# sczhou/CodeFormer

Measured on NVIDIA H100. Metric: faces_per_sec_512x512_batch32, higher is better.
Workload: dtype f32 (split-fp16 operands on tensor cores, fp32 accumulate)

## Files before the change

codeformer_b200/_lib.py:

```python
import ctypes
import os
from ctypes import POINTER, Structure, c_char_p, c_double, c_float, c_int, c_int32, c_int64, c_void_p

_HERE = os.path.dirname(os.path.abspath(__file__))
LIB_PATH = os.path.join(_HERE, 'libcfb200.so')


class CfbConfig(Structure):
    _fields_ = [('kind', c_int32), ('img_size', c_int32), ('nf', c_int32), ('n_ch_mult', c_int32),
                ('ch_mult', c_int32 * 8), ('res_blocks', c_int32), ('n_attn_res', c_int32),
                ('attn_res', c_int32 * 4), ('codebook_size', c_int32), ('emb_dim', c_int32), ('beta', c_float),
                ('dim_embd', c_int32), ('n_head', c_int32), ('n_layers', c_int32), ('latent_size', c_int32),
                ('n_connect', c_int32), ('connect', c_int32 * 6)]


_P = c_void_p
SIGNATURES = {
    'cfb_version': (c_int, []),
    'cfb_last_error': (c_char_p, []),
    'cfb_device_info': (c_int, [POINTER(c_int), POINTER(c_int), POINTER(c_int)]),
    'cfb_net_create': (c_void_p, [POINTER(CfbConfig)]),
    'cfb_net_destroy': (None, [_P]),
    'cfb_net_set_param': (c_int, [_P, c_char_p, _P, c_int64]),
    'cfb_net_prepare': (c_int, [_P, _P]),
# ... 54 lines not shown
    'cfb_retinaface_priors': (c_int64, [c_int32, c_int32]),
    'cfb_retinaface_create': (c_void_p, []),
    'cfb_retinaface_destroy': (None, [_P]),
    'cfb_retinaface_set_param': (c_int, [_P, c_char_p, _P, c_int64]),
    'cfb_retinaface_prepare': (c_int, [_P, _P]),
    'cfb_retinaface_workspace_bytes': (c_int64, [_P, c_int32, c_int32, c_int32]),
    'cfb_retinaface_forward': (c_int, [_P, _P, _P, _P, _P, c_int32, c_int32, c_int32, _P, c_int64, _P]),
    'cfb_retinaface_forward_u8': (c_int, [_P, _P, _P, _P, _P, c_int32, c_int32, c_int32, _P, c_int64, _P]),
    'cfb_retinaface_candidates': (c_int, [_P, _P, _P, c_int32, c_int32, c_int32, c_float, _P, _P, _P]),
    'cfb_yolov5face_predictions': (c_int64, [c_int32, c_int32]),
    'cfb_yolov5face_create': (c_void_p, []),
    'cfb_yolov5face_destroy': (None, [_P]),
    'cfb_yolov5face_set_param': (c_int, [_P, c_char_p, _P, c_int64]),
    'cfb_yolov5face_prepare': (c_int, [_P, _P]),
    'cfb_yolov5face_workspace_bytes': (c_int64, [_P, c_int32, c_int32, c_int32]),
    'cfb_yolov5face_forward': (c_int, [_P, _P, _P, _P, _P, _P, c_int32, c_int32, c_int32, _P, c_int64, _P]),
    'cfb_yolov5face_forward_u8': (c_int, [_P, _P, c_int32, c_int32, c_int32, c_int32, _P, _P, _P, _P, c_int32, c_int32, c_int32,
                                          _P, c_int64, _P]),
    'cfb_yolov5face_candidates': (c_int, [_P, c_int32, c_int32, c_int32, c_float, _P, _P, _P]),
    'cfb_check_async_status': (c_int, []),
    'cfb_debug_set_wait_limit': (c_int, [c_int64]),
    'cfb_debug_inject_fault': (c_int, [c_int32]),
    'cfb_debug_set_stamps': (c_int, [_P]),
    'cfb_nchw_to_nhwc': (c_int, [_P, _P, c_int32, c_int32, c_int32, _P]),
    'cfb_nhwc_to_nchw': (c_int, [_P, _P, c_int32, c_int32, c_int32, _P]),
    'cfb_warp_affine_u8': (c_int, [_P, c_int32, c_int32, _P, c_int32, _P, c_int32, c_int32, c_int32, c_int32, c_int32, c_int32, _P]),
    'cfb_resize_linear_u8': (c_int, [_P, c_int32, c_int32, c_int32, _P, c_int32, c_int32, _P]),
    'cfb_paste_faces_workspace_bytes': (c_int64, [c_int32, c_int32, c_int32, c_int32, c_int32, _P]),
    'cfb_paste_faces': (c_int, [_P, c_int32, c_int32, _P, c_int32, c_int32, _P, _P, c_double, _P, _P, _P, c_int64, _P]),
}

_lib = None


def load():
    global _lib
    if _lib is not None:
        return _lib
    if not os.path.exists(LIB_PATH):
        try:
            from . import build as _build
            _build.build(force=False)
        except Exception as e:
            raise RuntimeError(f'{LIB_PATH} is missing and could not be built with nvcc ({e}); there is no CPU or '
                               'PyTorch fallback for this path -- run `python -m codeformer_b200.build`') from e
    override = os.environ.get('CFB_LIB')
# ... 22 lines not shown
```

codeformer_b200/csrc/conv_tc.cu:

```cuda

#include <cuda.h>
#include <cuda_fp16.h>
#include <cuda_runtime.h>
#include <stdint.h>

#include <stdlib.h>

#include <atomic>
#include <mutex>

#include "conv_tc.cuh"

namespace cfb {

__global__ void tc_absmax_kernel(const float* __restrict__ w, int64_t total, unsigned* __restrict__ slot) {
  float m = 0.f;
  for (int64_t i = (int64_t)blockIdx.x * blockDim.x + threadIdx.x; i < total; i += (int64_t)gridDim.x * blockDim.x)
    m = fmaxf(m, fabsf(w[i]));
#pragma unroll
  for (int o = 16; o > 0; o >>= 1) m = fmaxf(m, __shfl_xor_sync(0xffffffffu, m, o));
  if ((threadIdx.x & 31) == 0) atomicMax(slot, __float_as_uint(m));
}

__global__ void tc_split_weights_kernel(const float* __restrict__ w, __half* __restrict__ hi, __half* __restrict__ lo,
// ... 241 lines not shown
  asm volatile(
      "cp.async.bulk.tensor.4d.shared::cluster.global.mbarrier::complete_tx::bytes [%0], [%1, {%3, %4, %5, %6}], [%2];"
      ::"r"(dst), "l"(map), "r"(bar), "r"(c0), "r"(c1), "r"(c2), "r"(c3)
      : "memory");
}
__device__ __forceinline__ void tma_load_3d(uint32_t dst, const CUtensorMap* map, uint32_t bar, int c0, int c1, int c2) {
  asm volatile(
      "cp.async.bulk.tensor.3d.shared::cluster.global.mbarrier::complete_tx::bytes [%0], [%1, {%3, %4, %5}], [%2];"
      ::"r"(dst), "l"(map), "r"(bar), "r"(c0), "r"(c1), "r"(c2)
      : "memory");
}
__device__ __forceinline__ bool elect_one() {
  uint32_t pred;
  asm volatile(
      "{\n\t.reg .b32 rx;\n\t.reg .pred px;\n\t"
      "elect.sync rx|px, 0xffffffff;\n\t"
      "selp.b32 %0, 1, 0, px;\n\t}"
      : "=r"(pred));
  return pred != 0;
}

__device__ __forceinline__ uint64_t wg_desc(uint32_t saddr, uint32_t sbo) {
  return (uint64_t)((saddr >> 4) & 0x3FFFu) | ((uint64_t)1 << 16) | ((uint64_t)((sbo >> 4) & 0x3FFFu) << 32) | ((uint64_t)1 << 62);
}
__device__ __forceinline__ void wg_fence() { asm volatile("wgmma.fence.sync.aligned;" ::: "memory"); }
__device__ __forceinline__ void wg_commit() { asm volatile("wgmma.commit_group.sync.aligned;" ::: "memory"); }
__device__ __forceinline__ void wg_wait_all() { asm volatile("wgmma.wait_group.sync.aligned 0;" ::: "memory"); }
__device__ __forceinline__ void wg_mma_64x64(float (&d)[32], uint64_t da, uint64_t db, uint32_t accum) {
  asm volatile(
      "{\n\t.reg .pred p;\n\t"
      "setp.ne.b32 p, %34, 0;\n\t"
      "wgmma.mma_async.sync.aligned.m64n64k16.f32.f16.f16 "
      "{%0, %1, %2, %3, %4, %5, %6, %7, %8, %9, %10, %11, %12, %13, %14, %15, "
      "%16, %17, %18, %19, %20, %21, %22, %23, %24, %25, %26, %27, %28, %29, %30, %31}, %32, %33, p, 1, 1, 0, 0;\n\t}"
      : "+f"(d[0]), "+f"(d[1]), "+f"(d[2]), "+f"(d[3]), "+f"(d[4]), "+f"(d[5]), "+f"(d[6]), "+f"(d[7]), "+f"(d[8]),
        "+f"(d[9]), "+f"(d[10]), "+f"(d[11]), "+f"(d[12]), "+f"(d[13]), "+f"(d[14]), "+f"(d[15]), "+f"(d[16]),
        "+f"(d[17]), "+f"(d[18]), "+f"(d[19]), "+f"(d[20]), "+f"(d[21]), "+f"(d[22]), "+f"(d[23]), "+f"(d[24]),
        "+f"(d[25]), "+f"(d[26]), "+f"(d[27]), "+f"(d[28]), "+f"(d[29]), "+f"(d[30]), "+f"(d[31])
      : "l"(da), "l"(db), "r"(accum)
      : "memory");
}

__device__ __forceinline__ void wg_mma_64x128(float (&d)[64], uint64_t da, uint64_t db, uint32_t accum) {
  asm volatile(
      "{\n\t.reg .pred p;\n\t"
      "setp.ne.b32 p, %66, 0;\n\t"
// ... 158 lines not shown
  int in_act;
  const float* bias;
  const float* residual;
  int out_act;
  const float* sft_dec;
  const float* sft_scale;
  float sft_w;
  const float* wscale_inv;
  float* out;
  __half* pl_hi;
  __half* pl_lo;
  float* gn_part;
  int gn_cpg;
#if CFB_TC_STAMPS
  long long* dbg;
#endif
};
#if CFB_TC_STAMPS
#define TC_STAMP(i) do { if (p.dbg != nullptr && blockIdx.x == 0) p.dbg[i] = clock64(); } while (0)
#else
#define TC_STAMP(i) do { } while (0)
#endif

constexpr int XF_SKEW = 128;
constexpr int TC_A_BYTES = 128 * 128;

template <int BN>
struct TcCfg {
  static_assert(BN == 64 || BN == 128, "the wgmma engine runs 64- or 128-wide n-tiles");
  static constexpr bool WIDE = BN == 128;
  static constexpr int MMA_WARPS = WIDE ? 8 : 4;
  static constexpr int EPI_WARPS = WIDE ? 4 : 8;
  static constexpr int THREADS = 32 * (MMA_WARPS + 1 + EPI_WARPS);
  static constexpr int B_BYTES = BN * 128;
  static constexpr int STAGE_BYTES = 2 * TC_A_BYTES + 2 * B_BYTES;
  static constexpr int STAGES = 3;
  static constexpr int SLOT_PITCH = BN + 4;
  static constexpr int SLOT_BYTES = 128 * SLOT_PITCH * 4;
  static constexpr int SLOTS = 1;
  static constexpr int STG_BYTES = WIDE ? 0 : 8 * 4096;
  static constexpr int TAIL_BYTES = SLOT_BYTES + 1024  + 512  + STG_BYTES;
  static constexpr int SMEM_BYTES = STAGES * STAGE_BYTES + TAIL_BYTES;
  static constexpr int H_A_PLANE = 23 * 1024;
  static constexpr int H_A_SLOT = 2 * H_A_PLANE;
  static constexpr int H_A_SLOTS = 2;
  static constexpr int H_B_SLOT = 2 * B_BYTES;
  static constexpr int H_B_SLOTS = WIDE ? 2 : 4;
  static constexpr int H_SMEM_BYTES = H_A_SLOTS * H_A_SLOT + H_B_SLOTS * H_B_SLOT + TAIL_BYTES;
  static constexpr int XF_WARPS = WIDE ? 2 : 4;
  static constexpr int XF_THREADS = THREADS + 32 * XF_WARPS + 32;
  static constexpr int X_A_SLOTS = 2;
  static constexpr int X_A_PLANE2 = H_A_PLANE + XF_SKEW;
  static constexpr int X_B_SLOTS = H_B_SLOTS;
  static constexpr int X_SMEM_BYTES = X_A_SLOTS * H_A_SLOT + X_B_SLOTS * H_B_SLOT + TAIL_BYTES;
};

template <int BN, int CPG, bool HALO, bool XF, bool GEN = false, bool K1 = false, bool CM = false, bool SILU = false>
__global__ void __launch_bounds__(XF ? TcCfg<BN>::XF_THREADS : TcCfg<BN>::THREADS, 1)
conv_tc_kernel(const __grid_constant__ CUtensorMap tmA_hi, const __grid_constant__ CUtensorMap tmA_lo,
               const __grid_constant__ CUtensorMap tmB_hi, const __grid_constant__ CUtensorMap tmB_lo, const TcParams p) {
  static_assert(!XF || HALO, "the fused operand transform exists for the halo engine only");
  static_assert(!GEN || (XF && CPG == 0), "the generalised addressing exists for the fused-transform engine only");
  static_assert(!K1 || (XF && !GEN && CPG == 0), "K1 = fused transform of a 1x1 conv (patch = tile): its own instantiation");
  using Cfg = TcCfg<BN>;
  constexpr bool WIDE = Cfg::WIDE;
  static_assert(!WIDE || (HALO && !GEN && !K1 && CPG != 2), "128-wide tiles exist for the 3x3 / Upsample halo engine");
  static_assert(!CM || (BN == 64 && HALO && !GEN && !K1), "channel-major tiles exist for the 64-channel 3x3 / Upsample halo convs");
  constexpr int MMA_WARPS = Cfg::MMA_WARPS, EPI_WARPS = Cfg::EPI_WARPS;
  constexpr int A_SLOTS = XF ? Cfg::X_A_SLOTS : Cfg::H_A_SLOTS;
  constexpr int STAGES = Cfg::STAGES;
// ... 2 lines not shown
  const int tile_step = (int)gridDim.x;
  extern __shared__ uint8_t smem_raw[];
  uint8_t* smem = reinterpret_cast<uint8_t*>((reinterpret_cast<uintptr_t>(smem_raw) + 1023) & ~(uintptr_t)1023);
  constexpr int NRING = HALO ? (XF ? Cfg::X_B_SLOTS : Cfg::H_B_SLOTS) : STAGES;
  constexpr int RING_BYTES = HALO ? Cfg::H_B_SLOT : STAGE_BYTES;
  uint8_t* ring_base = HALO ? smem + A_SLOTS * Cfg::H_A_SLOT : smem;
  float* acc_slot = reinterpret_cast<float*>(ring_base + NRING * RING_BYTES);
  uint64_t* bars = reinterpret_cast<uint64_t*>(ring_base + NRING * RING_BYTES + Cfg::SLOT_BYTES);
  uint64_t* full = bars;
  uint64_t* empty = bars + NRING;
  uint64_t* cfull = bars + 2 * NRING;
  uint64_t* cempty = bars + 2 * NRING + Cfg::SLOTS;
  uint64_t* afull = bars + 2 * NRING + 2 * Cfg::SLOTS;
  uint64_t* aempty = afull + 3;
  uint64_t* araw = aempty + 3;
  uint8_t* stage_buf = reinterpret_cast<uint8_t*>(bars) + 512;

  constexpr int NWARPS = (XF ? Cfg::XF_THREADS : Cfg::THREADS) / 32;
  const int pwarp = __shfl_sync(0xffffffffu, (int)(threadIdx.x >> 5), 0);
  const int ridx = NWARPS - 1 - pwarp;
  const int warp = pwarp < MMA_WARPS ? 1 : (ridx == 0 ? 0 : ridx + 1);
  const int lane = threadIdx.x & 31;
  bool aborted = false;
  if (threadIdx.x == 0) TC_STAMP(0);

  if (warp == 0 && lane == 0) {
    for (int a = 0; a < 3; ++a) {
      mbar_init(smem_u32(afull + a), XF ? Cfg::XF_WARPS : 1);
      mbar_init(smem_u32(aempty + a), MMA_WARPS);
      mbar_init(smem_u32(araw + a), 1);
    }
    asm volatile("prefetch.tensormap [%0];" ::"l"(&tmA_hi) : "memory");
    asm volatile("prefetch.tensormap [%0];" ::"l"(&tmA_lo) : "memory");
    asm volatile("prefetch.tensormap [%0];" ::"l"(&tmB_hi) : "memory");
    asm volatile("prefetch.tensormap [%0];" ::"l"(&tmB_lo) : "memory");
    for (int s = 0; s < NRING; ++s) { mbar_init(smem_u32(full + s), 1); mbar_init(smem_u32(empty + s), MMA_WARPS); }
    for (int a = 0; a < Cfg::SLOTS; ++a) {
      mbar_init(smem_u32(cfull + a), MMA_WARPS);
      mbar_init(smem_u32(cempty + a), EPI_WARPS);
    }
    asm volatile("fence.mbarrier_init.release.cluster;" ::: "memory");
  }
  __syncthreads();
  pdl_launch_dependents();
  pdl_wait();
  if (threadIdx.x == 0) TC_STAMP(1);

  const int total_tiles = p.m_tiles * p.n_tiles;
  const int nk = p.taps * p.kblocks;

  if (warp == 0) {
    {
      int stage = 0;
      uint32_t phase = 0;
      int aslot = 0;
      uint32_t aphase = 0;
      for (int tile = first_tile; tile < total_tiles; tile += tile_step) {
        const int mt = tile / p.n_tiles, nt = tile - mt * p.n_tiles;
        const int mtl = p.up4 ? (mt >> 2) : mt;
        const int par_y = p.up4 ? ((mt & 3) >> 1) : 0, par_x = p.up4 ? (mt & 1) : 0;
        const int per_img = p.tiles_x * p.tiles_y;
        const int n = mtl / per_img;
        const int rem = mtl - n * per_img;
        const int ty = rem / p.tiles_x, tx = rem - ty * p.tiles_x;
        const int y0 = ty * p.BH * p.stride, x0 = tx * p.BW * p.stride;
        if constexpr (HALO) {
          for (int kb = 0; kb < p.kblocks; ++kb) {
            if constexpr (!XF) {
              mbar_wait<500>(smem_u32(aempty + aslot), aphase ^ 1, aborted); if (aborted) goto teardown;
              if (elect_one()) {
                const uint32_t sa = smem_u32(smem + aslot * Cfg::H_A_SLOT);
                const uint32_t ab = smem_u32(afull + aslot);
                mbar_expect_tx(ab, (uint32_t)(2 * p.PW * p.PH * 128));
                tma_load_4d(sa, &tmA_hi, ab, kb * 64, x0 - p.pad, y0 - p.pad, n);
                tma_load_4d(sa + Cfg::H_A_PLANE, &tmA_lo, ab, kb * 64, x0 - p.pad, y0 - p.pad, n);
              }
              __syncwarp();
              if (++aslot == A_SLOTS) { aslot = 0; aphase ^= 1; }
            }
            for (int tap = 0; tap < p.taps; ++tap) {
              const int btap = p.up4 ? (mt & 3) * 4 + tap : tap;
              mbar_wait<500>(smem_u32(empty + stage), phase ^ 1, aborted); if (aborted) goto teardown;
              if (elect_one()) {
                if (tile == first_tile && tap == 0 && kb == 0) TC_STAMP(2);
                const uint32_t sb = smem_u32(ring_base + stage * RING_BYTES);
                const uint32_t fb = smem_u32(full + stage);
                const bool drop = p.fault && blockIdx.x == 0 && tile == first_tile && kb == 0 && tap == 0;
                mbar_expect_tx(fb, (uint32_t)Cfg::H_B_SLOT);
                if (!drop) tma_load_3d(sb, &tmB_hi, fb, kb * 64, nt * BN, btap);
                tma_load_3d(sb + Cfg::B_BYTES, &tmB_lo, fb, kb * 64, nt * BN, btap);
              }
              __syncwarp();
              if (++stage == NRING) { stage = 0; phase ^= 1; }
            }
          }
        } else {
          for (int tap = 0; tap < p.taps; ++tap) {
            int r, s, btap = tap;
            if (p.up4) { r = (tap >> 1) + par_y; s = (tap & 1) + par_x; btap = (mt & 3) * 4 + tap; }
            else { r = (p.taps == 9) ? tap / 3 : 0; s = (p.taps == 9) ? tap - r * 3 : 0; }
            for (int kb = 0; kb < p.kblocks; ++kb) {
              mbar_wait<500>(smem_u32(empty + stage), phase ^ 1, aborted); if (aborted) goto teardown;
              if (elect_one()) {
                if (tile == first_tile && tap == 0 && kb == 0) TC_STAMP(2);
                const uint32_t sa = smem_u32(smem + stage * STAGE_BYTES);
                const int hh = p.heads > 1 ? n % p.heads : 0, nimg = p.heads > 1 ? n / p.heads : n;
                const int a_img = p.a_img_per_head ? n : nimg;
                const int ac = p.a_c0 + hh * p.a_c_head + kb * 64, bc = p.b_c0 + hh * p.b_c_head + kb * 64;
                const int brow = nt * BN + hh * p.b_r_head;
                const int b3 = p.b_batched ? nimg : btap;
                const uint32_t fb = smem_u32(full + stage);
                const bool drop = p.fault && blockIdx.x == 0 && tile == first_tile && kb == 0 && tap == 0;
                mbar_expect_tx(fb, (uint32_t)Cfg::STAGE_BYTES);
                tma_load_4d(sa, &tmA_hi, fb, ac, x0 + s - p.pad, y0 + r - p.pad, a_img);
                tma_load_4d(sa + TC_A_BYTES, &tmA_lo, fb, ac, x0 + s - p.pad, y0 + r - p.pad, a_img);
                if (!drop) tma_load_3d(sa + 2 * TC_A_BYTES, &tmB_hi, fb, bc, brow, b3);
                tma_load_3d(sa + 2 * TC_A_BYTES + Cfg::B_BYTES, &tmB_lo, fb, bc, brow, b3);
              }
              __syncwarp();
              if (++stage == STAGES) { stage = 0; phase ^= 1; }
            }
          }
        }
      }
    }
  } else if (warp == 1) {
    {
      constexpr bool N128 = WIDE || CM;
      constexpr int MH = N128 ? 1 : 2;
      const uint32_t a_sbo = HALO ? (uint32_t)(p.PW * 128) : 1024u;
      const uint32_t a_half = HALO ? (uint32_t)(8 * p.PW * 128) : 8192u;
      const int wq = (int)(threadIdx.x >> 5) & 3;
      const int wg = (int)(threadIdx.x >> 7);
      const uint32_t bar_id = 2u + (uint32_t)wg;
      const uint32_t slot_base = smem_u32(acc_slot);
      int stage = 0;
      uint32_t phase = 0;
      int slot = 0;
      uint32_t slot_phase = 0;
      int aslot = 0;
      uint32_t aphase = 0;
      float acc[MH][N128 ? 64 : 32];
      if constexpr (N128) {
        for (int tile = first_tile; tile < total_tiles; tile += tile_step) {
          const int par = p.up4 ? ((tile / p.n_tiles) & 3) : 0;
          const int par_y = par >> 1, par_x = par & 1;
          for (int c0 = 0; c0 < nk; c0 += p.chunk) {
            const int c1 = min(c0 + p.chunk, nk);
            uint32_t prev_empty = 0, prev_aempty = 0;
            for (int it = c0; it < c1; ++it) {
              const int kb = it / p.taps;
              const int tap = it - kb * p.taps;
              if (tap == 0) {
                mbar_wait(smem_u32(afull + aslot), aphase, aborted);
                if (wg_any(aborted, bar_id)) { wg_wait_all(); aborted = true; goto teardown; }
              }
              int r = (p.taps == 9) ? tap / 3 : 0;
              int sft = (p.taps == 9) ? tap - r * 3 : 0;
              if (p.up4) { r = (tap >> 1) + par_y; sft = (tap & 1) + par_x; }
              const uint32_t a_hi0 = smem_u32(smem + aslot * Cfg::H_A_SLOT) + (uint32_t)((r * p.PW + sft) * 128) +
                                     (uint32_t)wg * a_half;
              const uint32_t a_lo0 = a_hi0 + (uint32_t)(XF ? Cfg::X_A_PLANE2 : Cfg::H_A_PLANE);
              const uint32_t bsm = smem_u32(ring_base + stage * RING_BYTES);
              mbar_wait(smem_u32(full + stage), phase, aborted);
              if (wg_any(aborted, bar_id)) { wg_wait_all(); aborted = true; goto teardown; }
              wg_fence();
#pragma unroll
              for (int k = 0; k < 4; ++k) {
                const uint64_t db_hi = wg_desc(bsm + 32 * k, 1024u), db_lo = wg_desc(bsm + Cfg::B_BYTES + 32 * k, 1024u);
                const uint64_t da_hi = wg_desc(a_hi0 + 32 * k, a_sbo), da_lo = wg_desc(a_lo0 + 32 * k, a_sbo);
                if constexpr (CM) {
                  wg_mma_64x128(acc[0], db_hi, da_lo, (it == c0 && k == 0) ? 0u : 1u);
                  wg_mma_64x128(acc[0], db_lo, da_hi, 1u);
                  wg_mma_64x128(acc[0], db_hi, da_hi, 1u);
                } else {
                  wg_mma_64x128(acc[0], da_lo, db_hi, (it == c0 && k == 0) ? 0u : 1u);
                  wg_mma_64x128(acc[0], da_hi, db_lo, 1u);
                  wg_mma_64x128(acc[0], da_hi, db_hi, 1u);
                }
              }
              wg_commit();
              wg_wait_1();
              __syncwarp();
              mbar_arrive_if(prev_empty, lane == 0 && prev_empty != 0);
              mbar_arrive_if(prev_aempty, lane == 0 && prev_aempty != 0);
              prev_empty = smem_u32(empty + stage);
              prev_aempty = tap == p.taps - 1 ? smem_u32(aempty + aslot) : 0u;
              if (++stage == NRING) { stage = 0; phase ^= 1; }
              if (tap == p.taps - 1 && ++aslot == A_SLOTS) { aslot = 0; aphase ^= 1; }
            }
            wg_wait_all();
            __syncwarp();
            mbar_arrive_if(prev_empty, lane == 0);
            mbar_arrive_if(prev_aempty, lane == 0 && prev_aempty != 0);
            if constexpr (CM) {
              mbar_wait(smem_u32(cempty + slot), slot_phase ^ 1, aborted);
              if (wg_any(aborted, bar_id)) { aborted = true; goto teardown; }
              const uint32_t st0 = slot_base + (uint32_t)(slot * Cfg::SLOT_BYTES) +
                                   (uint32_t)((2 * (lane & 3) * Cfg::SLOT_PITCH + wq * 16 + (lane >> 2)) * 4);
#pragma unroll
              for (int j = 0; j < 16; ++j) {
#pragma unroll
                for (int h8 = 0; h8 < 2; ++h8) {
#pragma unroll
                  for (int e = 0; e < 2; ++e) {
                    const uint32_t a = st0 + (uint32_t)(((8 * j + e) * Cfg::SLOT_PITCH + 8 * h8) * 4);
                    asm volatile("st.shared.f32 [%0], %1;" ::"r"(a), "f"(acc[0][4 * j + 2 * h8 + e]) : "memory");
                  }
                }
              }
              __syncwarp();
              if (lane == 0) mbar_arrive(smem_u32(cfull + slot));
              if (++slot == Cfg::SLOTS) { slot = 0; slot_phase ^= 1; }
              continue;
            }
            const bool first_chunk = c0 == 0;
            if (first_chunk) {
              mbar_wait(smem_u32(cempty + slot), slot_phase ^ 1, aborted);
              if (wg_any(aborted, bar_id)) { aborted = true; goto teardown; }
            }
            const uint32_t sbase = slot_base + (uint32_t)(slot * Cfg::SLOT_BYTES);
            const int row = wg * 64 + wq * 16 + (lane >> 2);
#pragma unroll
            for (int j = 0; j < 16; ++j) {
#pragma unroll
              for (int h8 = 0; h8 < 2; ++h8) {
                const uint32_t e = sbase + (uint32_t)(((row + 8 * h8) * Cfg::SLOT_PITCH + 8 * j + 2 * (lane & 3)) * 4);
                float x = 0.f, y = 0.f;
                if (!first_chunk) asm volatile("ld.shared.v2.f32 {%0, %1}, [%2];" : "=f"(x), "=f"(y) : "r"(e) : "memory");
                x = __fadd_rn(x, acc[0][4 * j + 2 * h8]);
                y = __fadd_rn(y, acc[0][4 * j + 2 * h8 + 1]);
                asm volatile("st.shared.v2.f32 [%0], {%1, %2};" ::"r"(e), "f"(x), "f"(y) : "memory");
              }
            }
          }
          if constexpr (!CM) {
            __syncwarp();
            if (lane == 0) mbar_arrive(smem_u32(cfull + slot));
            if (++slot == Cfg::SLOTS) { slot = 0; slot_phase ^= 1; }
          }
        }
      } else {
      for (int tile = first_tile; tile < total_tiles; tile += tile_step) {
        const int par = p.up4 ? ((tile / p.n_tiles) & 3) : 0;
        const int par_y = par >> 1, par_x = par & 1;
        for (int it = 0; it < nk; ++it) {
          uint32_t a_hi0, a_lo0, bsm;
          int tap = 0;
          if constexpr (HALO) {
            const int kb = it / p.taps;
            tap = it - kb * p.taps;
            if (tap == 0) { mbar_wait(smem_u32(afull + aslot), aphase, aborted); if (wg_any(aborted)) { aborted = true; goto teardown; } }
            int r = (p.taps == 9) ? tap / 3 : 0;
            int sft = (p.taps == 9) ? tap - r * 3 : 0;
            if (p.up4) { r = (tap >> 1) + par_y; sft = (tap & 1) + par_x; }
            const uint32_t aoff = (uint32_t)((r * p.PW + sft) * 128);
            a_hi0 = smem_u32(smem + aslot * Cfg::H_A_SLOT) + aoff;
            a_lo0 = a_hi0 + (uint32_t)(XF ? Cfg::X_A_PLANE2 : Cfg::H_A_PLANE);
            bsm = smem_u32(ring_base + stage * RING_BYTES);
          } else {
            a_hi0 = smem_u32(smem + stage * STAGE_BYTES);
            a_lo0 = a_hi0 + TC_A_BYTES;
            bsm = a_hi0 + 2 * TC_A_BYTES;
          }
// ... 408 lines not shown
              *reinterpret_cast<float2*>(gp + (colq / CPG) * 2) = make_float2(s0, q0);
            }
          }
        }
        __syncwarp();
      }
      }
      if constexpr (WIDE) {
        if (lane == 0) mbar_arrive(smem_u32(cempty + slot));
        if (++slot == Cfg::SLOTS) { slot = 0; slot_phase ^= 1; }
      }
      if (warp == 2 && lane == 0 && tile == first_tile) TC_STAMP(16);
      if (warp == 2 && lane == 0 && tile == first_tile + tile_step) TC_STAMP(18);
    }
    if (omax > 65504.f) report_overflow();
    if (warp == 2 && lane == 0) TC_STAMP(13);
  }

teardown:
  if (aborted) {
    const long long t0 = clock64();
    while (clock64() - t0 < 400000) {}
  }
  __syncthreads();
  if (threadIdx.x == 0) TC_STAMP(8);
}

int tc_bind_status_word(unsigned* host_mapped_dev_ptr, long long wait_limit_cycles) {
  const unsigned zero = 0;
  CFB_CUDA(cudaMemcpyToSymbol(g_status_host, &host_mapped_dev_ptr, sizeof(host_mapped_dev_ptr)));
  CFB_CUDA(cudaMemcpyToSymbol(g_wait_limit, &wait_limit_cycles, sizeof(wait_limit_cycles)));
  CFB_CUDA(cudaMemcpyToSymbol(g_abort, &zero, sizeof(zero)));
  return 0;
}
static std::atomic<int> g_inject_fault{0};
static std::atomic<long long*> g_stamps{nullptr};
int tc_set_stamps(long long* dev_ptr) { g_stamps.store(dev_ptr); return 0; }
int tc_inject_fault(int kind) { g_inject_fault.store(kind); return 0; }
int tc_clear_abort() {
  const unsigned zero = 0;
  CFB_CUDA(cudaMemcpyToSymbol(g_abort, &zero, sizeof(zero)));
  return 0;
}

typedef CUresult (*EncodeTiledFn)(CUtensorMap*, CUtensorMapDataType, cuuint32_t, void*, const cuuint64_t*, const cuuint64_t*,
                                  const cuuint32_t*, const cuuint32_t*, CUtensorMapInterleave, CUtensorMapSwizzle,
                                  CUtensorMapL2promotion, CUtensorMapFloatOOBfill);

static EncodeTiledFn get_encode_fn() {
  static EncodeTiledFn fn = nullptr;
  static std::once_flag once;
  std::call_once(once, [] {
    void* p = nullptr;
    cudaDriverEntryPointQueryResult q;
    if (cudaGetDriverEntryPoint("cuTensorMapEncodeTiled", &p, cudaEnableDefault, &q) == cudaSuccess &&
        q == cudaDriverEntryPointSuccess)
      fn = (EncodeTiledFn)p;
  });
  return fn;
}

static int make_map(CUtensorMap* m, const void* base, int rank, const uint64_t* dims, const uint64_t* strides_bytes,
                    const uint32_t* box, int spatial_stride = 1, bool f32 = false) {
  EncodeTiledFn fn = get_encode_fn();
  CFB_REQUIRE(fn != nullptr, "cuTensorMapEncodeTiled is not available from the driver");
  cuuint32_t estr[5] = {1, (cuuint32_t)spatial_stride, (cuuint32_t)spatial_stride, 1, 1};
  const CUresult rc = fn(m, f32 ? CU_TENSOR_MAP_DATA_TYPE_FLOAT32 : CU_TENSOR_MAP_DATA_TYPE_FLOAT16, (cuuint32_t)rank, const_cast<void*>(base),
                         reinterpret_cast<const cuuint64_t*>(dims), reinterpret_cast<const cuuint64_t*>(strides_bytes),
                         reinterpret_cast<const cuuint32_t*>(box), estr, CU_TENSOR_MAP_INTERLEAVE_NONE,
                         CU_TENSOR_MAP_SWIZZLE_128B, CU_TENSOR_MAP_L2_PROMOTION_L2_256B, CU_TENSOR_MAP_FLOAT_OOB_FILL_NONE);
  CFB_REQUIRE(rc == CUDA_SUCCESS, "cuTensorMapEncodeTiled failed (" + std::to_string((int)rc) + ")");
  return 0;
}

static inline int tile_bw(int W) {
  int bw = 1;
  while (bw < W && bw < 128) bw <<= 1;
  return bw;
}

static int tc_chunk_kblocks() {
  static int v = [] {
    const char* e = getenv("CFB_TC_CHUNK");
    int c = e ? atoi(e) : 8;
    return c < 1 ? 1 : (c > 4096 ? 4096 : c);
  }();
  return v;
}

static bool halo_enabled() {
  static bool v = [] { const char* e = getenv("CFB_TC_HALO"); return !(e && atoi(e) == 0); }();
  return v;
}
// ... 171 lines not shown
    const uint32_t box[4] = {32, (uint32_t)PW, (uint32_t)PH, 1};
    {
      const uint64_t dims[4] = {(uint64_t)C0, (uint64_t)Wp, (uint64_t)Hp, (uint64_t)a.N};
      const uint64_t str[3] = {(uint64_t)C0 * 4, (uint64_t)Wp * C0 * 4, (uint64_t)Hp * Wp * C0 * 4};
      CFB_CHECK(make_map(&mA_hi, a.in, 4, dims, str, box, 1, true));
    }
    {
      const uint64_t dims[4] = {(uint64_t)C1, (uint64_t)Wp, (uint64_t)Hp, (uint64_t)a.N};
      const uint64_t str[3] = {(uint64_t)C1 * 4, (uint64_t)Wp * C1 * 4, (uint64_t)Hp * Wp * C1 * 4};
      CFB_CHECK(make_map(&mA_lo, a.in2 ? a.in2 : a.in, 4, dims, str, box, 1, true));
    }
  } else {
    const int sp = a.mode == CONV_DOWN ? 2 : 1;
    const uint64_t dims[4] = {(uint64_t)a.Cin, (uint64_t)Wp, (uint64_t)Hp, (uint64_t)a.N};
    const uint64_t str[3] = {(uint64_t)a.Cin * 2, (uint64_t)Wp * a.Cin * 2, (uint64_t)Hp * Wp * a.Cin * 2};
    const uint32_t box[4] = {64, (uint32_t)(geo.halo ? PW : BW * sp), (uint32_t)(geo.halo ? PH : BH * sp), 1};
    CFB_CHECK(make_map(&mA_hi, hi, 4, dims, str, box, sp));
    CFB_CHECK(make_map(&mA_lo, lo, 4, dims, str, box, sp));
  }
  {
    const int taps = a.mode == CONV_UP ? 16 : a.ksize * a.ksize;
    const uint64_t dims[3] = {(uint64_t)a.Cin, (uint64_t)a.Cout, (uint64_t)taps};
    const uint64_t str[2] = {(uint64_t)a.Cin * 2, (uint64_t)a.Cout * a.Cin * 2};
    const uint32_t box[3] = {64, (uint32_t)BN, 1};
    CFB_CHECK(make_map(&mB_hi, a.wgt_hi, 3, dims, str, box));
    CFB_CHECK(make_map(&mB_lo, a.wgt_lo, 3, dims, str, box));
  }
  TcParams p;
  p.N = a.N; p.Ho = a.Ho; p.Wo = a.Wo; p.Cout = a.Cout;
  p.taps = a.ksize * a.ksize; p.pad = a.mode == CONV_DOWN ? a.down_pad : a.ksize / 2; p.stride = a.mode == CONV_DOWN ? 2 : 1;
  p.up4 = a.mode == CONV_UP ? 1 : 0;
  p.a_c0 = 0; p.b_c0 = 0; p.b_batched = 0;
  p.heads = 1; p.a_c_head = 0; p.b_c_head = 0; p.a_img_per_head = 0; p.b_r_head = 0; p.out_per_head = 1; p.o_c_head = 0;
  if (p.up4) { p.taps = 4; p.pad = 1; }
  p.chunk = tc_chunk_kblocks();
  p.PW = PW; p.PH = PH;
  p.BW = BW; p.BH = BH;
  p.tiles_x = ((p.up4 ? a.W : a.Wo) + BW - 1) / BW; p.tiles_y = ((p.up4 ? a.H : a.Ho) + BH - 1) / BH;
  {
    int64_t lowres_tiles = (int64_t)a.N * p.tiles_x * p.tiles_y;
    p.m_tiles = (int)(lowres_tiles * (p.up4 ? 4 : 1));
  }
  p.n_tiles = a.Cout / BN; p.kblocks = a.Cin / 64;
  p.Hin = Hp; p.Win = Wp; p.pad_mode = a.pad_mode; p.sub = a.subsample ? 1 : 0;
  p.out_pitch = a.out_pitch ? a.out_pitch : a.Cout; p.out_c0 = a.out_c0; p.cout_valid = a.cout_valid ? a.cout_valid : a.Cout;
  p.res_pitch = a.res_pitch ? a.res_pitch : p.out_pitch; p.residual2 = a.residual2;
  p.res2_pitch = a.res2_pitch ? a.res2_pitch : p.out_pitch; p.post_scale = a.post_scale;
  if (a.gen) {
    CFB_REQUIRE(a.xform && !a.gn_part && !a.out_planes && !a.sft_dec, "conv_tc: generalised variant = fused transform, fp32 output only");
// ... 470 lines not shown
```

codeformer_b200/csrc/kernels.cuh:

```cuda
#pragma once
#include <cuda_runtime.h>
#include <stdint.h>
#include <string>

namespace cfb {

void set_error(const std::string& msg);
#define CFB_CUDA(expr)                                                                            \
  do {                                                                                            \
    cudaError_t _e = (expr);                                                                      \
    if (_e != cudaSuccess) {                                                                      \
      ::cfb::set_error(std::string(#expr) + ": " + cudaGetErrorString(_e) + " @" + __FILE__ + ":" + \
                       std::to_string(__LINE__));                                                 \
      return 1;                                                                                   \
    }                                                                                             \
  } while (0)
#define CFB_LAUNCH_CHECK()                                                                        \
  do {                                                                                            \
    cudaError_t _e = cudaGetLastError();                                                          \
    if (_e != cudaSuccess) {                                                                      \
      ::cfb::set_error(std::string("kernel launch failed: ") + cudaGetErrorString(_e) + " @" +    \
                       __FILE__ + ":" + std::to_string(__LINE__));                                \
      return 1;                                                                                   \
    }                                                                                             \
    ::cfb::count_launch();                                                                        \
  } while (0)
#define CFB_CHECK(x)                                                                              \
  do {                                                                                            \
    if ((x) != 0) return 1;                                                                       \
  } while (0)
#define CFB_REQUIRE(cond, msg)                                                                    \
  do {                                                                                            \
    if (!(cond)) {                                                                                \
      ::cfb::set_error(std::string(msg) + " [" #cond "] @" + __FILE__ + ":" + std::to_string(__LINE__)); \
      return 1;                                                                                   \
    }                                                                                             \
  } while (0)

#define CFB_STATUS_TIMEOUT 1u
#define CFB_STATUS_OVERFLOW 2u
int async_status_init(cudaStream_t st);
int async_status_check(const char* where);
int tc_bind_status_word(unsigned* host_mapped_dev_ptr, long long wait_limit_cycles);
int tc_clear_abort();
int tc_set_stamps(long long* dev_ptr);
int tc_inject_fault(int kind);

void count_launch();
int64_t launch_count();
void reset_launch_count();

bool pdl_enabled();
#ifdef __CUDACC__
#ifndef CFB_PDL_DEVICE
#define CFB_PDL_DEVICE 1
#endif
#if CFB_PDL_DEVICE
__device__ __forceinline__ void pdl_wait() { asm volatile("griddepcontrol.wait;" ::: "memory"); }
__device__ __forceinline__ void pdl_launch_dependents() { asm volatile("griddepcontrol.launch_dependents;" ::: "memory"); }
#else
__device__ __forceinline__ void pdl_wait() {}
__device__ __forceinline__ void pdl_launch_dependents() {}
#endif
template <typename... KArgs, typename... Args>
inline cudaError_t launch_pdl(void (*kernel)(KArgs...), dim3 grid, dim3 block, size_t smem, cudaStream_t st, Args&&... args) {
  cudaLaunchConfig_t cfg = {};
  cfg.gridDim = grid; cfg.blockDim = block; cfg.dynamicSmemBytes = smem; cfg.stream = st;
  cudaLaunchAttribute attr[1];
// ... 149 lines not shown
```

codeformer_b200/csrc/runtime.cu:

```cuda
#include <cuda_fp16.h>
#include <cuda_runtime.h>
#include <stdint.h>
#include <string.h>

#include <algorithm>
#include <array>
#include <atomic>
#include <cmath>
#include <map>
#include <mutex>
#include <string>
#include <unordered_map>
#include <vector>

#include "../../include/cfb200.h"
#include "kernels.cuh"
#include "conv_tc.cuh"

namespace cfb {

static thread_local std::string g_err;
void set_error(const std::string& msg) { g_err = msg; }
const std::string& last_error() { return g_err; }
static std::atomic<int64_t> g_launches{0};
// ... 2411 lines not shown
  CFB_CHECK(cfb::async_status_init(nullptr));
  {
    std::lock_guard<std::mutex> lk(cfb::g_status_mu);
    cfb::g_wait_limit_cycles = cycles;
  }
  int dev = 0;
  CFB_CUDA(cudaGetDevice(&dev));
  unsigned* dptr = nullptr;
  CFB_CUDA(cudaHostGetDevicePointer((void**)&dptr, cfb::g_status_words, 0));
  return cfb::tc_bind_status_word(dptr + dev, cycles);
  API_END(1)
}

int cfb_debug_inject_fault(int32_t kind) {
  API_BEGIN
  return cfb::tc_inject_fault(kind);
  API_END(1)
}
int cfb_debug_set_stamps(int64_t* stamps) {
  API_BEGIN
  return cfb::tc_set_stamps((long long*)stamps);
  API_END(1)
}

int cfb_net_set_param(cfb_net* n, const char* name, const float* dev_ptr, int64_t numel) {
  API_BEGIN
  CFB_REQUIRE(n && name && dev_ptr, "cfb_net_set_param: NULL argument");
  std::lock_guard<std::mutex> lk(n->mu);
  n->raw[name] = {dev_ptr, numel};
  n->prepared = false;
  return 0;
  API_END(1)
}

int cfb_net_prepare(cfb_net* n, void* stream) {
  API_BEGIN
  CFB_REQUIRE(n, "cfb_net_prepare: NULL net");
  std::lock_guard<std::mutex> lk(n->mu);
  return cfb::prepare(n, (cudaStream_t)stream);
  API_END(1)
}

int64_t cfb_workspace_bytes(cfb_net* n, int32_t batch) {
  API_BEGIN
  if (!n) { cfb::set_error("cfb_workspace_bytes: NULL net"); return -1; }
  std::lock_guard<std::mutex> lk(n->mu);
// ... 508 lines not shown
```

include/cfb200.h:

```cpp
#ifndef CFB200_H_
#define CFB200_H_

#include <stdint.h>

#ifdef __cplusplus
extern "C" {
#endif

#define CFB_VERSION 100

typedef struct cfb_net cfb_net;

typedef struct cfb_config {
  int32_t kind;
  int32_t img_size;
  int32_t nf;
  int32_t n_ch_mult;
  int32_t ch_mult[8];
  int32_t res_blocks;
  int32_t n_attn_res;
  int32_t attn_res[4];
  int32_t codebook_size;
  int32_t emb_dim;
  float   beta;
// ... 131 lines not shown
                                    int32_t batch, int32_t h, int32_t w, void* workspace, int64_t workspace_bytes, void* stream);
int       cfb_retinaface_candidates(const float* loc, const float* conf, const float* landms, int32_t batch, int32_t h, int32_t w,
                                    float conf_threshold, float* rows, int32_t* counts, void* stream);

typedef struct cfb_yolov5face cfb_yolov5face;
int64_t         cfb_yolov5face_predictions(int32_t h, int32_t w);
cfb_yolov5face* cfb_yolov5face_create(void);
void            cfb_yolov5face_destroy(cfb_yolov5face* net);
int             cfb_yolov5face_set_param(cfb_yolov5face* net, const char* name, const float* dev_ptr, int64_t numel);
int             cfb_yolov5face_prepare(cfb_yolov5face* net, void* stream);
int64_t         cfb_yolov5face_workspace_bytes(cfb_yolov5face* net, int32_t batch, int32_t h, int32_t w);
int             cfb_yolov5face_forward(cfb_yolov5face* net, const float* x_nchw, float* pred, float* raw0, float* raw1, float* raw2,
                                       int32_t batch, int32_t h, int32_t w, void* workspace, int64_t workspace_bytes, void* stream);
int             cfb_yolov5face_forward_u8(cfb_yolov5face* net, const uint8_t* img_bgr_hwc, int32_t img_h, int32_t img_w, int32_t top,
                                          int32_t left, float* pred, float* raw0, float* raw1, float* raw2, int32_t batch, int32_t h,
                                          int32_t w, void* workspace, int64_t workspace_bytes, void* stream);
int             cfb_yolov5face_candidates(const float* pred, int32_t batch, int32_t h, int32_t w, float conf_threshold, float* rows,
                                          int32_t* counts, void* stream);

int cfb_check_async_status(void);
int cfb_debug_set_wait_limit(int64_t cycles);
int cfb_debug_inject_fault(int32_t kind);
int cfb_debug_set_stamps(int64_t* stamps);
int cfb_nchw_to_nhwc(const float* in, float* out, int32_t n, int32_t c, int32_t hw, void* stream);
int cfb_nhwc_to_nchw(const float* in, float* out, int32_t n, int32_t c, int32_t hw, void* stream);

int cfb_warp_affine_u8(const uint8_t* img, int32_t h, int32_t w, const double* affines, int32_t n, uint8_t* out,
                       int32_t out_h, int32_t out_w, int32_t border_mode, int32_t v0, int32_t v1, int32_t v2, void* stream);
int cfb_resize_linear_u8(const uint8_t* src, int32_t n, int32_t h, int32_t w, uint8_t* dst, int32_t out_h, int32_t out_w,
                         void* stream);
int64_t cfb_paste_faces_workspace_bytes(int32_t h_up, int32_t w_up, int32_t n, int32_t face_size, int32_t use_parse,
                                        const double* inverse_affines);
int cfb_paste_faces(uint8_t* canvas, int32_t h_up, int32_t w_up, const uint8_t* faces, int32_t n, int32_t face_size,
                    const uint8_t* parse_masks, const double* inverse_affines, double upscale, float* debug_canvas,
                    int32_t* w_edge_out, void* workspace, int64_t workspace_bytes, void* stream);

#ifdef __cplusplus
}
#endif
#endif
```

Measured before the change: 138.5.

## Split wide-tile weight loads into half-K stages with 64B swizzle

For 128-wide n-tiles, each 64-deep K block of weights is now loaded as two 32-deep halves using a 64-byte swizzle TMA map. The ring gets four smaller B slots, and the MMA warpgroup waits on and releases each half separately. The aim is finer-grained overlap between weight TMA and wgmma, with less smem per slot, at the cost of more barrier traffic and more commit/wait points per K block. Optional stall-cycle counters are also added, compiled out by default, behind a new debug API.

```diff
diff --git a/codeformer_b200/_lib.py b/codeformer_b200/_lib.py
--- a/codeformer_b200/_lib.py
+++ b/codeformer_b200/_lib.py
@@ -100,6 +100,7 @@
     'cfb_debug_set_wait_limit': (c_int, [c_int64]),
     'cfb_debug_inject_fault': (c_int, [c_int32]),
     'cfb_debug_set_stamps': (c_int, [_P]),
+    'cfb_debug_tc_stalls': (c_int, [_P, c_int32, c_int32]),
     'cfb_nchw_to_nhwc': (c_int, [_P, _P, c_int32, c_int32, c_int32, _P]),
     'cfb_nhwc_to_nchw': (c_int, [_P, _P, c_int32, c_int32, c_int32, _P]),
     'cfb_warp_affine_u8': (c_int, [_P, c_int32, c_int32, _P, c_int32, _P, c_int32, c_int32, c_int32, c_int32, c_int32, c_int32, _P]),
diff --git a/codeformer_b200/csrc/conv_tc.cu b/codeformer_b200/csrc/conv_tc.cu
--- a/codeformer_b200/csrc/conv_tc.cu
+++ b/codeformer_b200/csrc/conv_tc.cu
@@ -287,6 +287,9 @@
 
 __device__ __forceinline__ uint64_t wg_desc(uint32_t saddr, uint32_t sbo) {
   return (uint64_t)((saddr >> 4) & 0x3FFFu) | ((uint64_t)1 << 16) | ((uint64_t)((sbo >> 4) & 0x3FFFu) << 32) | ((uint64_t)1 << 62);
+}
+__device__ __forceinline__ uint64_t wg_desc_sw64(uint32_t saddr) {
+  return (uint64_t)((saddr >> 4) & 0x3FFFu) | ((uint64_t)1 << 16) | ((uint64_t)(512u >> 4) << 32) | ((uint64_t)2 << 62);
 }
 __device__ __forceinline__ void wg_fence() { asm volatile("wgmma.fence.sync.aligned;" ::: "memory"); }
 __device__ __forceinline__ void wg_commit() { asm volatile("wgmma.commit_group.sync.aligned;" ::: "memory"); }
@@ -491,6 +494,37 @@
 #define TC_STAMP(i) do { } while (0)
 #endif
 
+#ifndef CFB_TC_STALLS
+#define CFB_TC_STALLS 0
+#endif
+enum TcStall {
+  TC_STALL_FULL = 0,
+  TC_STALL_AFULL,
+  TC_STALL_CEMPTY,
+  TC_STALL_FOLD,
+  TC_STALL_MMA_TOTAL,
+  TC_STALL_EMPTY,
+  TC_STALL_TMA_TOTAL,
+  TC_STALL_COUNT
+};
+#if CFB_TC_STALLS
+__device__ unsigned long long g_tc_stalls[TC_STALL_COUNT];
+struct TcStalls {
+  long long c[TC_STALL_COUNT] = {};
+  __device__ __forceinline__ long long now() const { return clock64(); }
+  __device__ __forceinline__ void add(int i, long long t0) { c[i] += clock64() - t0; }
+  __device__ __forceinline__ void flush() {
+    for (int i = 0; i < TC_STALL_COUNT; ++i) atomicAdd(&g_tc_stalls[i], (unsigned long long)c[i]);
+  }
+};
+#else
+struct TcStalls {
+  __device__ __forceinline__ long long now() const { return 0; }
+  __device__ __forceinline__ void add(int, long long) {}
+  __device__ __forceinline__ void flush() {}
+};
+#endif
+
 constexpr int XF_SKEW = 128;
 constexpr int TC_A_BYTES = 128 * 128;
 
@@ -513,8 +547,11 @@
   static constexpr int H_A_PLANE = 23 * 1024;
   static constexpr int H_A_SLOT = 2 * H_A_PLANE;
   static constexpr int H_A_SLOTS = 2;
-  static constexpr int H_B_SLOT = 2 * B_BYTES;
-  static constexpr int H_B_SLOTS = WIDE ? 2 : 4;
+  static constexpr int H_B_SPLIT = WIDE ? 2 : 1;
+  static constexpr int H_B_KCH = 64 / H_B_SPLIT;
+  static constexpr int H_B_PLANE = BN * H_B_KCH * 2;
+  static constexpr int H_B_SLOT = 2 * H_B_PLANE;
+  static constexpr int H_B_SLOTS = 4;
   static constexpr int H_SMEM_BYTES = H_A_SLOTS * H_A_SLOT + H_B_SLOTS * H_B_SLOT + TAIL_BYTES;
   static constexpr int XF_WARPS = WIDE ? 2 : 4;
   static constexpr int XF_THREADS = THREADS + 32 * XF_WARPS + 32;
@@ -563,6 +600,7 @@
   const int warp = pwarp < MMA_WARPS ? 1 : (ridx == 0 ? 0 : ridx + 1);
   const int lane = threadIdx.x & 31;
   bool aborted = false;
+  TcStalls stalls;
   if (threadIdx.x == 0) TC_STAMP(0);
 
   if (warp == 0 && lane == 0) {
@@ -592,6 +630,7 @@
 
   if (warp == 0) {
     {
+      const long long t_role = stalls.now();
       int stage = 0;
       uint32_t phase = 0;
       int aslot = 0;
@@ -621,18 +660,25 @@
             }
             for (int tap = 0; tap < p.taps; ++tap) {
               const int btap = p.up4 ? (mt & 3) * 4 + tap : tap;
-              mbar_wait<500>(smem_u32(empty + stage), phase ^ 1, aborted); if (aborted) goto teardown;
-              if (elect_one()) {
-                if (tile == first_tile && tap == 0 && kb == 0) TC_STAMP(2);
-                const uint32_t sb = smem_u32(ring_base + stage * RING_BYTES);
-                const uint32_t fb = smem_u32(full + stage);
-                const bool drop = p.fault && blockIdx.x == 0 && tile == first_tile && kb == 0 && tap == 0;
-                mbar_expect_tx(fb, (uint32_t)Cfg::H_B_SLOT);
-                if (!drop) tma_load_3d(sb, &tmB_hi, fb, kb * 64, nt * BN, btap);
-                tma_load_3d(sb + Cfg::B_BYTES, &tmB_lo, fb, kb * 64, nt * BN, btap);
+#pragma unroll
+              for (int h = 0; h < Cfg::H_B_SPLIT; ++h) {
+                const long long t_w = stalls.now();
+                mbar_wait<500>(smem_u32(empty + stage), phase ^ 1, aborted);
+                stalls.add(TC_STALL_EMPTY, t_w);
+                if (aborted) goto teardown;
+                if (elect_one()) {
+                  if (tile == first_tile && tap == 0 && kb == 0 && h == 0) TC_STAMP(2);
+                  const uint32_t sb = smem_u32(ring_base + stage * RING_BYTES);
+                  const uint32_t fb = smem_u32(full + stage);
+                  const bool drop = p.fault && blockIdx.x == 0 && tile == first_tile && kb == 0 && tap == 0 && h == 0;
+                  const int kc = kb * 64 + h * Cfg::H_B_KCH;
+                  mbar_expect_tx(fb, (uint32_t)Cfg::H_B_SLOT);
+                  if (!drop) tma_load_3d(sb, &tmB_hi, fb, kc, nt * BN, btap);
+                  tma_load_3d(sb + Cfg::H_B_PLANE, &tmB_lo, fb, kc, nt * BN, btap);
+                }
+                __syncwarp();
+                if (++stage == NRING) { stage = 0; phase ^= 1; }
               }
-              __syncwarp();
-              if (++stage == NRING) { stage = 0; phase ^= 1; }
             }
           }
         } else {
@@ -664,6 +710,7 @@
           }
         }
       }
+      stalls.add(TC_STALL_TMA_TOTAL, t_role);
     }
   } else if (warp == 1) {
     {
@@ -683,6 +730,7 @@
       uint32_t aphase = 0;
       float acc[MH][N128 ? 64 : 32];
       if constexpr (N128) {
+        const long long t_role = stalls.now();
         for (int tile = first_tile; tile < total_tiles; tile += tile_step) {
           const int par = p.up4 ? ((tile / p.n_tiles) & 3) : 0;
           const int par_y = par >> 1, par_x = par & 1;
@@ -693,7 +741,9 @@
               const int kb = it / p.taps;
               const int tap = it - kb * p.taps;
               if (tap == 0) {
+                const long long t_w = stalls.now();
                 mbar_wait(smem_u32(afull + aslot), aphase, aborted);
+                stalls.add(TC_STALL_AFULL, t_w);
                 if (wg_any(aborted, bar_id)) { wg_wait_all(); aborted = true; goto teardown; }
               }
               int r = (p.taps == 9) ? tap / 3 : 0;
@@ -702,40 +752,53 @@
               const uint32_t a_hi0 = smem_u32(smem + aslot * Cfg::H_A_SLOT) + (uint32_t)((r * p.PW + sft) * 128) +
                                      (uint32_t)wg * a_half;
               const uint32_t a_lo0 = a_hi0 + (uint32_t)(XF ? Cfg::X_A_PLANE2 : Cfg::H_A_PLANE);
-              const uint32_t bsm = smem_u32(ring_base + stage * RING_BYTES);
-              mbar_wait(smem_u32(full + stage), phase, aborted);
-              if (wg_any(aborted, bar_id)) { wg_wait_all(); aborted = true; goto teardown; }
-              wg_fence();
-#pragma unroll
-              for (int k = 0; k < 4; ++k) {
-                const uint64_t db_hi = wg_desc(bsm + 32 * k, 1024u), db_lo = wg_desc(bsm + Cfg::B_BYTES + 32 * k, 1024u);
-                const uint64_t da_hi = wg_desc(a_hi0 + 32 * k, a_sbo), da_lo = wg_desc(a_lo0 + 32 * k, a_sbo);
-                if constexpr (CM) {
-                  wg_mma_64x128(acc[0], db_hi, da_lo, (it == c0 && k == 0) ? 0u : 1u);
-                  wg_mma_64x128(acc[0], db_lo, da_hi, 1u);
-                  wg_mma_64x128(acc[0], db_hi, da_hi, 1u);
-                } else {
-                  wg_mma_64x128(acc[0], da_lo, db_hi, (it == c0 && k == 0) ? 0u : 1u);
-                  wg_mma_64x128(acc[0], da_hi, db_lo, 1u);
-                  wg_mma_64x128(acc[0], da_hi, db_hi, 1u);
+              constexpr int KS = 4 / Cfg::H_B_SPLIT;
+#pragma unroll
+              for (int h = 0; h < Cfg::H_B_SPLIT; ++h) {
+                const uint32_t bsm = smem_u32(ring_base + stage * RING_BYTES);
+                const long long t_w = stalls.now();
+                mbar_wait(smem_u32(full + stage), phase, aborted);
+                stalls.add(TC_STALL_FULL, t_w);
+                if (wg_any(aborted, bar_id)) { wg_wait_all(); aborted = true; goto teardown; }
+                wg_fence();
+#pragma unroll
+                for (int ks = 0; ks < KS; ++ks) {
+                  const int k = h * KS + ks;
+                  const uint64_t da_hi = wg_desc(a_hi0 + 32 * k, a_sbo), da_lo = wg_desc(a_lo0 + 32 * k, a_sbo);
+                  if constexpr (CM) {
+                    const uint64_t db_hi = wg_desc(bsm + 32 * ks, 1024u), db_lo = wg_desc(bsm + Cfg::H_B_PLANE + 32 * ks, 1024u);
+                    wg_mma_64x128(acc[0], db_hi, da_lo, (it == c0 && k == 0) ? 0u : 1u);
+                    wg_mma_64x128(acc[0], db_lo, da_hi, 1u);
+                    wg_mma_64x128(acc[0], db_hi, da_hi, 1u);
+                  } else {
+                    const uint64_t db_hi = wg_desc_sw64(bsm + 32 * ks), db_lo = wg_desc_sw64(bsm + Cfg::H_B_PLANE + 32 * ks);
+                    wg_mma_64x128(acc[0], da_lo, db_hi, (it == c0 && k == 0) ? 0u : 1u);
+                    wg_mma_64x128(acc[0], da_hi, db_lo, 1u);
+                    wg_mma_64x128(acc[0], da_hi, db_hi, 1u);
+                  }
                 }
+                wg_commit();
+                wg_wait_1();
+                __syncwarp();
+                mbar_arrive_if(prev_empty, lane == 0 && prev_empty != 0);
+                mbar_arrive_if(prev_aempty, lane == 0 && prev_aempty != 0);
+                prev_empty = smem_u32(empty + stage);
+                prev_aempty = (h == Cfg::H_B_SPLIT - 1 && tap == p.taps - 1) ? smem_u32(aempty + aslot) : 0u;
+                if (++stage == NRING) { stage = 0; phase ^= 1; }
               }
-              wg_commit();
-              wg_wait_1();
-              __syncwarp();
-              mbar_arrive_if(prev_empty, lane == 0 && prev_empty != 0);
-              mbar_arrive_if(prev_aempty, lane == 0 && prev_aempty != 0);
-              prev_empty = smem_u32(empty + stage);
-              prev_aempty = tap == p.taps - 1 ? smem_u32(aempty + aslot) : 0u;
-              if (++stage == NRING) { stage = 0; phase ^= 1; }
               if (tap == p.taps - 1 && ++aslot == A_SLOTS) { aslot = 0; aphase ^= 1; }
             }
+            long long t_fold = stalls.now();
             wg_wait_all();
             __syncwarp();
             mbar_arrive_if(prev_empty, lane == 0);
             mbar_arrive_if(prev_aempty, lane == 0 && prev_aempty != 0);
             if constexpr (CM) {
+              stalls.add(TC_STALL_FOLD, t_fold);
+              const long long t_w = stalls.now();
               mbar_wait(smem_u32(cempty + slot), slot_phase ^ 1, aborted);
+              stalls.add(TC_STALL_CEMPTY, t_w);
+              t_fold = stalls.now();
               if (wg_any(aborted, bar_id)) { aborted = true; goto teardown; }
               const uint32_t st0 = slot_base + (uint32_t)(slot * Cfg::SLOT_BYTES) +
                                    (uint32_t)((2 * (lane & 3) * Cfg::SLOT_PITCH + wq * 16 + (lane >> 2)) * 4);
@@ -753,11 +816,16 @@
               __syncwarp();
               if (lane == 0) mbar_arrive(smem_u32(cfull + slot));
               if (++slot == Cfg::SLOTS) { slot = 0; slot_phase ^= 1; }
+              stalls.add(TC_STALL_FOLD, t_fold);
               continue;
             }
             const bool first_chunk = c0 == 0;
             if (first_chunk) {
+              stalls.add(TC_STALL_FOLD, t_fold);
+              const long long t_w = stalls.now();
               mbar_wait(smem_u32(cempty + slot), slot_phase ^ 1, aborted);
+              stalls.add(TC_STALL_CEMPTY, t_w);
+              t_fold = stalls.now();
               if (wg_any(aborted, bar_id)) { aborted = true; goto teardown; }
             }
             const uint32_t sbase = slot_base + (uint32_t)(slot * Cfg::SLOT_BYTES);
@@ -774,6 +842,7 @@
                 asm volatile("st.shared.v2.f32 [%0], {%1, %2};" ::"r"(e), "f"(x), "f"(y) : "memory");
               }
             }
+            stalls.add(TC_STALL_FOLD, t_fold);
           }
           if constexpr (!CM) {
             __syncwarp();
@@ -781,6 +850,7 @@
             if (++slot == Cfg::SLOTS) { slot = 0; slot_phase ^= 1; }
           }
         }
+        stalls.add(TC_STALL_MMA_TOTAL, t_role);
       } else {
       for (int tile = first_tile; tile < total_tiles; tile += tile_step) {
         const int par = p.up4 ? ((tile / p.n_tiles) & 3) : 0;
@@ -1235,6 +1305,7 @@
     const long long t0 = clock64();
     while (clock64() - t0 < 400000) {}
   }
+  if ((warp == 1 && (threadIdx.x & 127) == 0) || (warp == 0 && lane == 0)) stalls.flush();
   __syncthreads();
   if (threadIdx.x == 0) TC_STAMP(8);
 }
@@ -1249,6 +1320,22 @@
 static std::atomic<int> g_inject_fault{0};
 static std::atomic<long long*> g_stamps{nullptr};
 int tc_set_stamps(long long* dev_ptr) { g_stamps.store(dev_ptr); return 0; }
+int tc_read_stalls(long long* host, int n, bool reset) {
+#if CFB_TC_STALLS
+  CFB_REQUIRE(n >= 0 && n <= TC_STALL_COUNT, "tc_read_stalls: at most TC_STALL_COUNT counters");
+  CFB_CUDA(cudaDeviceSynchronize());
+  if (n > 0) CFB_CUDA(cudaMemcpyFromSymbol(host, g_tc_stalls, (size_t)n * sizeof(long long)));
+  if (reset) {
+    const unsigned long long zero[TC_STALL_COUNT] = {};
+    CFB_CUDA(cudaMemcpyToSymbol(g_tc_stalls, zero, sizeof(zero)));
+  }
+  return 0;
+#else
+  (void)host; (void)n; (void)reset;
+  CFB_REQUIRE(false, "stall counters exist only in builds with -DCFB_TC_STALLS=1");
+  return 1;
+#endif
+}
 int tc_inject_fault(int kind) { g_inject_fault.store(kind); return 0; }
 int tc_clear_abort() {
   const unsigned zero = 0;
@@ -1274,14 +1361,15 @@
 }
 
 static int make_map(CUtensorMap* m, const void* base, int rank, const uint64_t* dims, const uint64_t* strides_bytes,
-                    const uint32_t* box, int spatial_stride = 1, bool f32 = false) {
+                    const uint32_t* box, int spatial_stride = 1, bool f32 = false,
+                    CUtensorMapSwizzle swizzle = CU_TENSOR_MAP_SWIZZLE_128B) {
   EncodeTiledFn fn = get_encode_fn();
   CFB_REQUIRE(fn != nullptr, "cuTensorMapEncodeTiled is not available from the driver");
   cuuint32_t estr[5] = {1, (cuuint32_t)spatial_stride, (cuuint32_t)spatial_stride, 1, 1};
   const CUresult rc = fn(m, f32 ? CU_TENSOR_MAP_DATA_TYPE_FLOAT32 : CU_TENSOR_MAP_DATA_TYPE_FLOAT16, (cuuint32_t)rank, const_cast<void*>(base),
                          reinterpret_cast<const cuuint64_t*>(dims), reinterpret_cast<const cuuint64_t*>(strides_bytes),
                          reinterpret_cast<const cuuint32_t*>(box), estr, CU_TENSOR_MAP_INTERLEAVE_NONE,
-                         CU_TENSOR_MAP_SWIZZLE_128B, CU_TENSOR_MAP_L2_PROMOTION_L2_256B, CU_TENSOR_MAP_FLOAT_OOB_FILL_NONE);
+                         swizzle, CU_TENSOR_MAP_L2_PROMOTION_L2_256B, CU_TENSOR_MAP_FLOAT_OOB_FILL_NONE);
   CFB_REQUIRE(rc == CUDA_SUCCESS, "cuTensorMapEncodeTiled failed (" + std::to_string((int)rc) + ")");
   return 0;
 }
@@ -1499,9 +1587,11 @@
     const int taps = a.mode == CONV_UP ? 16 : a.ksize * a.ksize;
     const uint64_t dims[3] = {(uint64_t)a.Cin, (uint64_t)a.Cout, (uint64_t)taps};
     const uint64_t str[2] = {(uint64_t)a.Cin * 2, (uint64_t)a.Cout * a.Cin * 2};
-    const uint32_t box[3] = {64, (uint32_t)BN, 1};
-    CFB_CHECK(make_map(&mB_hi, a.wgt_hi, 3, dims, str, box));
-    CFB_CHECK(make_map(&mB_lo, a.wgt_lo, 3, dims, str, box));
+    const bool half_kb = BN == 128;
+    const uint32_t box[3] = {half_kb ? 32u : 64u, (uint32_t)BN, 1};
+    const CUtensorMapSwizzle sw = half_kb ? CU_TENSOR_MAP_SWIZZLE_64B : CU_TENSOR_MAP_SWIZZLE_128B;
+    CFB_CHECK(make_map(&mB_hi, a.wgt_hi, 3, dims, str, box, 1, false, sw));
+    CFB_CHECK(make_map(&mB_lo, a.wgt_lo, 3, dims, str, box, 1, false, sw));
   }
   TcParams p;
   p.N = a.N; p.Ho = a.Ho; p.Wo = a.Wo; p.Cout = a.Cout;
diff --git a/codeformer_b200/csrc/kernels.cuh b/codeformer_b200/csrc/kernels.cuh
--- a/codeformer_b200/csrc/kernels.cuh
+++ b/codeformer_b200/csrc/kernels.cuh
@@ -44,6 +44,7 @@
 int tc_bind_status_word(unsigned* host_mapped_dev_ptr, long long wait_limit_cycles);
 int tc_clear_abort();
 int tc_set_stamps(long long* dev_ptr);
+int tc_read_stalls(long long* host, int n, bool reset);
 int tc_inject_fault(int kind);
 
 void count_launch();
diff --git a/codeformer_b200/csrc/runtime.cu b/codeformer_b200/csrc/runtime.cu
--- a/codeformer_b200/csrc/runtime.cu
+++ b/codeformer_b200/csrc/runtime.cu
@@ -2457,6 +2457,12 @@
   return cfb::tc_set_stamps((long long*)stamps);
   API_END(1)
 }
+int cfb_debug_tc_stalls(int64_t* counters, int32_t n, int32_t reset) {
+  API_BEGIN
+  CFB_REQUIRE(counters || n == 0, "cfb_debug_tc_stalls: NULL argument");
+  return cfb::tc_read_stalls((long long*)counters, n, reset != 0);
+  API_END(1)
+}
 
 int cfb_net_set_param(cfb_net* n, const char* name, const float* dev_ptr, int64_t numel) {
   API_BEGIN
diff --git a/include/cfb200.h b/include/cfb200.h
--- a/include/cfb200.h
+++ b/include/cfb200.h
@@ -177,6 +177,7 @@
 int cfb_debug_set_wait_limit(int64_t cycles);
 int cfb_debug_inject_fault(int32_t kind);
 int cfb_debug_set_stamps(int64_t* stamps);
+int cfb_debug_tc_stalls(int64_t* counters, int32_t n, int32_t reset);
 int cfb_nchw_to_nhwc(const float* in, float* out, int32_t n, int32_t c, int32_t hw, void* stream);
 int cfb_nhwc_to_nchw(const float* in, float* out, int32_t n, int32_t c, int32_t hw, void* stream);
 
```

Result: faster. 140.1, median of 6 (+1.1%).
